# mhx/dwarfs

Measured on AMD Instinct MI355X. Metric: ricepp encode+decode GiB/s, device-resident uint16 blocks, 1/2/4/8 GPUs, higher is better.
Workload: dtype u16; 1 GPU; 4096 independent 64 KiB uint16 blocks per GPU, ricepp bs128 cs1 BE ulsb0, encode+decode round trip (BASELINE.json configs[1]); blocks_per_gpu=4096, block_bytes=65536, parallelism=shard1 (blocks sharded, RCCL all-gather of encoded sizes), step_launch=eager

## Files before the change

### dwarfs_amd/csrc/ricepp_decode_fused.hip

```cpp
#include <hip/hip_runtime.h>
#include <stdint.h>

#include <algorithm>

#include "ricepp_amd.h"
#include "ricepp_internal.h"
#include "ricepp_stats.h"
#include "ricepp_tables.h"

#ifdef RPP_STATS
__device__ unsigned long long g_dec_stats[16];
#endif

namespace {

constexpr int kParsePrio = 1;

__device__ __forceinline__ uint4 tb_entry(const uint4* tb, uint32_t off16) {
  return *reinterpret_cast<const uint4*>(reinterpret_cast<const char*>(tb) + off16);
}

template <uint32_t CS, bool SH>
__global__ __launch_bounds__(kWave* kDecMaxWaves) void rpp_decode_kernel(DecParams p) {
  extern __shared__ __attribute__((aligned(16))) uint4 dsm[];
  const uint32_t b = blockIdx.x * p.waves + __builtin_amdgcn_readfirstlane(threadIdx.x / kWave);
  bool mine = b < p.nblocks;
  if (mine && p.only_fallback) mine = p.status[b] == rpp_internal::kSegFallback;
  if (mine && p.units && p.units[b] > 1) mine = false;
  if (!__syncthreads_or(mine)) return;
  copy_tables(dsm);
  __syncthreads();
  const uint4* tab = dsm;
  const uint32_t lane = lane_id();
  const uint32_t wv = __builtin_amdgcn_readfirstlane(threadIdx.x / kWave);
  uint32_t ring_w = kTabBytes / 4 + wv * kWaveLdsWords;
  asm("" : "+s"(ring_w));
  uint32_t* ring = reinterpret_cast<uint32_t*>(dsm) + ring_w;
  uint32_t* list = ring + kRingWords + kRingPad + kListLead;
  if (lane < kListLead) list[(int)lane - (int)kListLead] = 0u;
  const uint32_t bs = p.bs, be = p.be, ulsb = p.ulsb;
  const uint32_t selbe = be ? 0x02030001u : 0x03020100u;
  const uint32_t selpack = be ? 0x04050001u : 0x05040100u;
  const uint32_t lane24 = kSegBits * lane;
  if (!mine) return;
#ifdef RPP_STATS
  uint32_t stat_acc[16] = {0};
  unsigned long long tprev_;
  asm volatile("s_memtime %0\n\ts_waitcnt lgkmcnt(0)" : "=s"(tprev_)::"memory");
#endif

  int32_t status = RPP_OK;
  uint32_t N = 0, nbytes = 0, mis = 0;
  uint64_t nb_all = 0, lim_all = 0;
  const uint8_t* in = p.in;
  uint16_t* out = p.out;
  {
    const uint64_t n64 = p.n_samples[b];
    const uint64_t ioff = p.in_off[b];
    const uint64_t nb64 = p.in_bytes[b];
    if (n64 % CS != 0 || n64 >= RPP_MAX_STREAM_SAMPLES || nb64 >= (UINT64_C(1) << 32) - 8) {
      status = RPP_INVALID_ARGUMENT;
    } else {
      mis = (uint32_t)(ioff & 3u);
      N = (uint32_t)n64;
      nb_all = nb64 + mis;
      lim_all = 8u * mis + 64u * ((nb64 + 7u) >> 3);
      in = p.in + (ioff - mis);
      out = p.out + p.out_off[b];
    }
  }
  const bool aligned16 = ((uintptr_t)in & 15u) == 0;
  nbytes = (uint32_t)nb_all;
  uint32_t lim = (uint32_t)min(lim_all, (uint64_t)0xFFFFFFFFu);
  uint64_t base_w = 0;
  const uint32_t chunk_len = CS * bs;
  const uint32_t nchunks = status == RPP_OK ? (N + chunk_len - 1) / chunk_len : 0u;

  uint32_t fill_w = 0;
  bool pend = false;
  uint32_t vm_after = 0;
  auto retire = [&]() {
    if (pend) {
      vm_wait_all_but(vm_after);
      fill_w += kChunkWords;
      pend = false;
    }
  };
  auto refill_sync = [&]() {
    const uint32_t w = fill_w + 4 * lane;
    uint4 v;
    if (aligned16 && 4 * w + 16 <= nbytes) {
      v = *reinterpret_cast<const uint4*>(in + 4 * w);
    } else {
      v = make_uint4(stream_word(in, nbytes, w), stream_word(in, nbytes, w + 1), stream_word(in, nbytes, w + 2),
                     stream_word(in, nbytes, w + 3));
    }
    *reinterpret_cast<uint4*>(&ring[w & kRingMask]) = v;
    if ((w & kRingMask) < kRingPad) *reinterpret_cast<uint4*>(&ring[kRingWords + (w & kRingMask)]) = v;
    fill_w += kChunkWords;
  };
  auto request = [&]() {
    if (4u * (fill_w + kChunkWords) > nbytes) return;
    const uint32_t slot = __builtin_amdgcn_readfirstlane((uint32_t)(uintptr_t)&ring[fill_w & kRingMask]);
    const uint8_t* src = in + 4u * fill_w;
    if (aligned16) {
      glds16(src + 16u * lane, slot);
    } else {
#pragma unroll
      for (uint32_t q = 0; q < 4; ++q) glds4(src + 256u * q + 4u * lane, slot + 256u * q);
    }
    if ((fill_w & kRingMask) == 0)
      glds4(src + 4u * lane, __builtin_amdgcn_readfirstlane((uint32_t)(uintptr_t)&ring[kRingWords]));
    pend = true;
    vm_after = 0;
  };
  refill_sync();
  refill_sync();
  lds_fence();
  auto ensure = [&](uint32_t w) {
    if (fill_w < w + kAhead) {
      retire();
      while (fill_w < w + kAhead) refill_sync();
      lds_fence();
    }
  };
  auto wptr = [&](uint32_t w) -> const uint32_t* { return ring + (w & kRingMask); };
  auto peek32 = [&](uint32_t pos) -> uint32_t {
    const uint32_t* q = wptr(pos >> 5);
    return __builtin_amdgcn_alignbit(q[1], q[0], pos & 31u);
  };

  uint32_t last0 = 0, last1 = 0;
  uint32_t P = 8 * mis + 16 * CS;
  auto rebase = [&]() {
    if (P < (1u << 30)) return;
    const uint32_t sh = ((P >> 5) - kRingWords) & ~(kRingWords - 1u);
    in += 4ull * sh;
    base_w += sh;
    P -= 32u * sh;
    fill_w -= sh;
    nbytes = (uint32_t)(nb_all - 4ull * base_w);
    lim = (uint32_t)min(lim_all - 32ull * base_w, (uint64_t)0xFFFFFFFFu);
  };
  if (status == RPP_OK) {
    if (P > lim) status = RPP_TRUNCATED_INPUT;
    last0 = __builtin_amdgcn_readfirstlane(peek32(8 * mis) & 0xFFFFu);
    if (CS > 1) last1 = __builtin_amdgcn_readfirstlane(peek32(8 * mis + 16) & 0xFFFFu);
  }
  auto load_x = [&](uint32_t sb, uint32_t& xl, uint32_t& xh) {
    const uint32_t* q = wptr(sb >> 5);
    const uint32_t o = sb & 31u;
    const uint32_t a0 = q[0], a1 = q[1], a2 = q[2];
    xl = __builtin_amdgcn_alignbit(a1, a0, o);
    xh = __builtin_amdgcn_alignbit(a2, a1, o);
  };
  auto ring_keep = [&](uint32_t q) {
    if (pend && fill_w < (q >> 5) + kAhead + 128) retire();
    if (!pend && fill_w <= (q >> 5) + 766) request();
  };
  const uint32_t nsb = nchunks * CS;
  const bool fast_bs = bs == 2 * kWave ? (CS == 2 || (((uintptr_t)out) & 3u) == 0)
                                       : (bs == 16 || bs == 32 || bs == 64);
  const uint32_t nsb_fast = fast_bs ? (N / chunk_len) * CS : 0u;
  const uint32_t lane_off1 = lane < bs ? 2u * CS * lane : 0x7FFFFFF0u;
  const __amdgpu_buffer_rsrc_t orsrc = __builtin_amdgcn_make_buffer_rsrc(out, (short)0, (int)(2 * N), 0x00020000);
  ScanRegs sreg;

  for (uint32_t s = 0; s < nsb && status == RPP_OK; ++s) {
    rebase();
    auto fast = [&]<uint32_t MT, uint32_t LO, uint32_t HI, bool TWO>() {
      constexpr bool W32 = LO >= 8;
      constexpr uint32_t SB = W32 ? 32u : kSegBits;
      const uint32_t n = TWO ? 2 * kWave : bs;
      const uint4* const list4 = reinterpret_cast<const uint4*>(list);
      uint2* const list2 = reinterpret_cast<uint2*>(list);
      auto seg_bits = [&](uint32_t q, uint32_t& xh) {
        if constexpr (W32) {
          const uint32_t* w = ring + (((q >> 5) + lane) & kRingMask);
          const uint32_t w0 = w[0], w1 = w[1], w2 = w[2];
          xh = __builtin_amdgcn_alignbit(w2, w1, q & 31u);
          return __builtin_amdgcn_alignbit(w1, w0, q & 31u);
        } else {
          const uint32_t x = q + lane24;
          const uint32_t* w = ring + ((x >> 5) & kRingMask);
          xh = 0u;
          return __builtin_amdgcn_alignbit(w[1], w[0], x);
        }
      };
      auto fs_of = [](uint32_t h) { return (h & 15u) - 1u; };
      auto header_ok = [](uint32_t h) { return (uint32_t)((h & 15u) - (LO + 1) <= HI - LO); };
      auto parse = [&](uint32_t q, uint32_t xl, uint32_t xh, uint32_t fs, uint4 e0, uint4 e1, uint4 e2, uint4 e3,
                       uint32_t& Pe, uint32_t& xln, uint32_t& xhn, uint32_t rider, uint32_t& rider_incl,
                       auto&& mid) -> uint32_t {
        __builtin_amdgcn_s_setprio(kParsePrio);
        const uint32_t k = fs + 1;
        const uint32_t pe_base = q + 4u + n * k;
        uint32_t tm, cnt, incl;
        uint32_t tot2;
        if constexpr (!W32) {
          const Map8 M01 = comp8(Map8{e1.x, e1.y}, Map8{e0.x, e0.y});
          const Map8 M = comp8(Map8{e2.x, e2.y}, M01);
          auto scan_sel = [&]() {
            Map8 S = scan8_shr1(M, sreg.r1);
            S = scan8_shr2(S, sreg.r2);
            S = scan8_shr4(S, sreg.r4);
            S = scan8_shr8(S, sreg.r8);
            S = scan8_bc15(S, sreg.b15);
            S = scan8_bc31(S, sreg.b31);
            const Map8 X = shift8_wave(S, sreg.w1);
            return __builtin_amdgcn_perm(X.hi, X.lo, 0xFFFFFF04u);
          };
          auto term_mask = [&](uint32_t sel) {
            const uint32_t a0 = __builtin_amdgcn_perm(e0.w, e0.z, sel);
            const uint32_t a1 = __builtin_amdgcn_perm(e1.w, e1.z, __builtin_amdgcn_perm(e0.y, e0.x, sel));
            const uint32_t a2 = __builtin_amdgcn_perm(e2.w, e2.z, __builtin_amdgcn_perm(M01.hi, M01.lo, sel));
            return __builtin_amdgcn_perm(a2, __builtin_amdgcn_perm(a1, a0, 0x0C0C0400u), 0x0C040100u);
          };
          tm = term_mask(scan_sel());
          cnt = __builtin_popcount(tm);
          const uint32_t incl2 = wave_incl_sum(cnt | (rider << 16));
          incl = incl2 & 0xFFFFu;
          rider_incl = incl2 >> 16;
          tot2 = readlane(incl2, kWave - 1);
        } else {
          uint64_t finm;
          w32_count(e0, e1, e2, e3, n, rider, sreg, tm, cnt, incl, finm, rider_incl);
          tot2 = readlane(incl, kWave - 1) | (readlane(rider_incl, kWave - 1) << 16);
        }
        const uint32_t excl = incl - cnt;
        RPP_TSTAMP(7);
        uint32_t t[MT];
#pragma unroll
        for (uint32_t j = 0; j < MT; ++j) {
          t[j] = ffbl(tm);
          tm &= tm - 1;
        }
        RPP_TSTAMP(8);
        const uint32_t base = cnt != 0 && excl < n ? excl : 256u;
        uint32_t abase = (uint32_t)((int)(SB * lane - 4u) + __mul24((int)base, -(int)k));
        asm volatile("" : "+v"(abase));
        const uint32_t xr = xl >> 1;
#pragma unroll
        for (int j = MT - 1; j >= 0; --j) {
          const uint32_t rem = W32 ? __builtin_amdgcn_ubfe(__builtin_amdgcn_alignbit(xh, xl, t[j]), 1, fs)
                                   : __builtin_amdgcn_ubfe(xr, t[j], fs);
          list2[base + j] = make_uint2(abase + t[j] - j * k, rem);
          lds_fence();
        }
        Pe = pe_base + __builtin_amdgcn_readfirstlane(list[2 * (n - 1)]);
        __builtin_amdgcn_s_setprio(0);
        xln = seg_bits(Pe, xhn);
        mid(rider_incl, tot2 >> 16);
        RPP_TSTAMP(13);
        return (uint32_t)((tot2 & 0xFFFFu) >= n);
      };
      auto deltas = [&](uint4 tt, uint32_t aprev, uint32_t fs, uint32_t& d1, uint32_t& dsum) {
        if constexpr (TWO) {
          const uint32_t df0 = lshl_or(tt.x - aprev, fs, tt.y), df1 = lshl_or(tt.z - tt.x, fs, tt.w);
          const uint32_t d0 = (df0 >> 1) ^ neg_lsb(df0);
          d1 = (df1 >> 1) ^ neg_lsb(df1);
          dsum = d0 + d1;
        } else {
          const uint32_t df = lshl_or(tt.x - aprev, fs, tt.y);
          d1 = (df >> 1) ^ neg_lsb(df);
          dsum = lane < n ? d1 : 0u;
        }
      };
      auto store = [&](uint32_t d1, uint32_t inc, uint32_t inc_last, uint32_t sx) {
        const uint32_t comp = sx % CS;
        const uint32_t lastc = comp ? last1 : last0;
        const uint32_t v1 = lastc + inc;
        if constexpr (!TWO) {
          const uint32_t o = SH ? px_write2<true>(v1, selbe, ulsb) : __builtin_amdgcn_perm(v1, v1, selbe);
          __builtin_amdgcn_raw_buffer_store_b16((uint16_t)o, orsrc, lane_off1,
                                                (int)(2 * ((sx / CS) * chunk_len + comp)), 0);
          const uint32_t lnew = lastc + inc_last;
          if (comp) last1 = lnew;
          else last0 = lnew;
          return;
        }
        const uint32_t o = SH ? px_write2<true>(__builtin_amdgcn_perm(v1, v1 - d1, 0x05040100u), selbe, ulsb)
                              : __builtin_amdgcn_perm(v1, v1 - d1, selpack);
        if constexpr (CS == 1) {
          __builtin_amdgcn_raw_buffer_store_b32(o, orsrc, 4 * lane, (int)(sx * (2 * n)), 0);
        } else {
          const int sbase = (int)(2 * ((sx / CS) * chunk_len + comp));
          __builtin_amdgcn_raw_buffer_store_b16((uint16_t)o, orsrc, 4 * CS * lane, sbase, 0);
          __builtin_amdgcn_raw_buffer_store_b16((uint16_t)(o >> 16), orsrc, 4 * CS * lane + 2 * CS, sbase, 0);
        }
        const uint32_t lnew = lastc + inc_last;
        if (comp) last1 = lnew;
        else last0 = lnew;
      };
      auto lookups = [&](uint32_t xl, uint32_t fs, uint4& e0, uint4& e1, uint4& e2, uint4& e3) {
        const uint4* tb = tab + 256u * fs;
        e0 = tb_entry(tb, sdwa_byte16<0>(xl));
        e1 = tb_entry(tb, sdwa_byte16<1>(xl));
        e2 = tb_entry(tb, sdwa_byte16<2>(xl));
        if constexpr (W32) e3 = tb_entry(tb, sdwa_byte16<3>(xl));
        if constexpr (!W32) e3 = make_uint4(0u, 0u, 0u, 0u);
      };

      uint32_t pn_limit, trig_bits;
      auto ring_bounds = [&]() {
        pn_limit = __builtin_amdgcn_readfirstlane(min(min(lim - 4u, 32u * (fill_w - kAhead) + 31u), 1u << 31));
        trig_bits =
            __builtin_amdgcn_readfirstlane(32u * (pend ? fill_w - (kAhead + 127u) : (fill_w > 766u ? fill_w - 766u : 0u)));
      };
      constexpr uint32_t kStoresPerSub = TWO && CS == 2 ? 2u : 1u;
      uint32_t s_keep = s;
      ring_bounds();
      uint32_t Pn;
      uint32_t xh;
      uint32_t xl = seg_bits(P, xh);
      const uint32_t h = __builtin_amdgcn_readfirstlane(xl);
      uint32_t fs = fs_of(h);
      uint4 e0, e1, e2, e3;
      lookups(xl, fs, e0, e1, e2, e3);
      uint32_t unused_rider;
      uint32_t xlB, xhB;
      uint32_t ok =
          parse(P, xl, xh, fs, e0, e1, e2, e3, Pn, xlB, xhB, 0u, unused_rider, [](uint32_t, uint32_t) {}) & header_ok(h);
      uint32_t pn_read_limit = pn_limit;
      while (ok) {
        uint4 tt;
        uint32_t aprev;
        if constexpr (TWO) {
          tt = list4[lane];
          aprev = list[4 * lane - 2];
        } else {
          const uint2 t2 = list2[lane];
          tt = make_uint4(t2.x, t2.y, 0u, 0u);
          aprev = list[2 * lane - 2];
        }
        const uint32_t hB = __builtin_amdgcn_readfirstlane(xlB);
        RPP_TSTAMP(1);
        RPP_STAT(0, 1);
        uint32_t d1A, sumA, incA;
        const uint32_t nxt = (uint32_t)(s + 1 < nsb_fast) & (uint32_t)(Pn <= pn_read_limit) & header_ok(hB);
        pn_read_limit = pn_limit;
        const uint32_t fsB = fs_of(hB);
        lookups(xlB, fsB, e0, e1, e2, e3);
        deltas(tt, aprev, fs, d1A, sumA);
        RPP_TSTAMP(2);
        uint32_t PnB, xlC, xhC;
        ok = parse(Pn, xlB, xhB, fsB, e0, e1, e2, e3, PnB, xlC, xhC, sumA, incA,
                   [&](uint32_t inc, uint32_t inc_last) { store(d1A, inc, inc_last, s); });
        ++s;
        P = Pn;
        if (!(ok & nxt)) {
          if (P > lim) status = RPP_TRUNCATED_INPUT;
          break;
        }
        Pn = PnB;
        fs = fsB;
        xlB = xlC;
        xhB = xhC;
        if (Pn >= trig_bits) {
          vm_after += (s - s_keep) * kStoresPerSub;
          s_keep = s;
          ring_keep(Pn);
          ring_bounds();
        }
        RPP_TSTAMP(15);
      }
    };
    while (s < nsb_fast && status == RPP_OK && fill_w >= (P >> 5) + kAhead && P + 4 <= lim) {
      rebase();
      const uint32_t* w = ring + ((P >> 5) & kRingMask);
      const uint32_t h = __builtin_amdgcn_readfirstlane(__builtin_amdgcn_alignbit(w[1], w[0], P & 31u)) & 15u;
      const uint32_t s0 = s;
      if (bs == 2 * kWave) {
        if (h - 6u <= 2u) fast.template operator()<4, 5, 7, true>();
        else if (h - 3u <= 2u) fast.template operator()<8, 2, 4, true>();
        else if (h - 9u <= 5u) fast.template operator()<4, 8, 13, true>();
        else if (h == 2u) fast.template operator()<12, 1, 4, true>();
      } else {
        if (h - 6u <= 2u) fast.template operator()<4, 5, 7, false>();
        else if (h - 3u <= 2u) fast.template operator()<8, 2, 4, false>();
        else if (h - 9u <= 5u) fast.template operator()<4, 8, 13, false>();
        else if (h == 2u) fast.template operator()<12, 1, 4, false>();
      }
      last0 &= 0xFFFFu;
      last1 &= 0xFFFFu;
      if (s == s0) break;
    }
    if (s >= nsb || status != RPP_OK) break;
    vm_after = 0;
    const uint32_t comp = s % CS;
    const uint32_t cbase = (s / CS) * chunk_len;
    const uint32_t n = min(N - cbase, chunk_len) / CS;
    RPP_TSTAMP(4);
    ensure(P >> 5);
    if (P + 4 > lim) {
      status = RPP_TRUNCATED_INPUT;
      break;
    }
    uint32_t xl, xh;
    load_x(P + kSegBits * lane, xl, xh);
    const uint32_t fsp1 = __builtin_amdgcn_readfirstlane(xl) & 15u;
    const uint32_t P4 = P + 4;
    uint16_t* dst = out + cbase + comp;
    const bool dw = CS == 1 && (((uintptr_t)dst) & 3u) == 0;
    auto put2 = [&](uint32_t i0, uint32_t o, bool ok0, bool ok1) {
      if (dw && ok1) {
        *reinterpret_cast<uint32_t*>(dst + i0) = o;
      } else {
        if (ok0) dst[CS * i0] = (uint16_t)o;
        if (ok1) dst[CS * (i0 + 1)] = (uint16_t)(o >> 16);
      }
    };
    RPP_STAT(6, 1);
    RPP_TSTAMP(5);
    if (fsp1 == 0) {
      const uint32_t v = px_write(comp ? last1 : last0, be, ulsb) * 0x10001u;
      for (uint32_t i0 = 2 * lane; i0 < n; i0 += 2 * kWave) put2(i0, v, true, i0 + 1 < n);
      P = P4;
    } else if (fsp1 == 15) {
      if ((uint64_t)P4 + 16ull * n > lim) {
        status = RPP_TRUNCATED_INPUT;
        break;
      }
      for (uint32_t i0 = 2 * lane; i0 < n; i0 += 2 * kWave) {
        put2(i0, peek32(P4 + 16 * i0), true, i0 + 1 < n);
      }
      const uint32_t lv = __builtin_amdgcn_readfirstlane(px_read(peek32(P4 + 16 * (n - 1)) & 0xFFFFu, be, ulsb));
      if (comp) last1 = lv;
      else last0 = lv;
      P = P4 + 16 * n;
    } else {
      const uint32_t fs = fsp1 - 1;
      const uint32_t k = fsp1;
      const uint32_t fmask = (1u << fs) - 1u;
      const uint4* tb = tab + 256u * fs;
      uint32_t acc = comp ? last1 : last0, start = P4, xdone = 0;
      uint32_t held_i = 0xFFFFFFFFu, held_r = 0;
      auto extract = [&](uint32_t m) {
        for (; xdone < m; xdone += 2 * kWave) {
          const uint32_t i0 = xdone + 2 * lane;
          const bool ok0 = i0 < m, ok1 = i0 + 1 < m;
          const uint2 tt = *reinterpret_cast<const uint2*>(&list[min(i0, kListDump - 2)]);
          const uint32_t t0 = tt.x, t1 = ok1 ? tt.y : t0;
          const uint32_t st0 = dpp_keep<kDppWaveShr1>(start, t1 + k);
          const uint32_t r0 = i0 == held_i ? held_r : peek32(t0 + 1) & fmask, r1 = peek32(t1 + 1) & fmask;
          const uint32_t df0 = ((t0 - st0) << fs) | r0, df1 = ((t1 - t0 - k) << fs) | r1;
          const uint32_t d0 = ok0 ? (df0 >> 1) ^ (0u - (df0 & 1u)) : 0u;
          const uint32_t d1 = ok1 ? (df1 >> 1) ^ (0u - (df1 & 1u)) : 0u;
          const uint32_t inc = wave_incl_sum(d0 + d1);
          const uint32_t v1 = acc + inc;
          put2(i0, px_write2<true>(((v1 - d1) & 0xFFFFu) | (v1 << 16), selbe, ulsb), ok0, ok1);
          acc += wave_last(inc);
          start = wave_last(t1) + k;
        }
        xdone = m;
        start = __builtin_amdgcn_readfirstlane(list[m - 1]) + k;
      };
      uint32_t q0 = P, s0 = 4, done = 0;
      for (;;) {
        RPP_STAT(0, 1);
        const uint32_t sb = q0 + kSegBits * lane;
        const uint4 e0 = tb[xl & 0xFFu], e1 = tb[__builtin_amdgcn_ubfe(xl, 8, 8)],
                    e2 = tb[__builtin_amdgcn_ubfe(xl, 16, 8)];
        RPP_TSTAMP(10);
        uint32_t tm, xexit;
        if (fs < 8) {
          Map8 M = comp8(Map8{e2.x, e2.y}, comp8(Map8{e1.x, e1.y}, Map8{e0.x, e0.y}));
          M = scan_step8<kDppRowShr1>(M);
          M = scan_step8<kDppRowShr2>(M);
          M = scan_step8<kDppRowShr4>(M);
          M = scan_step8<kDppRowShr8>(M);
          M = scan_step8<kDppRowBcast15, 0xA>(M);
          M = scan_step8<kDppRowBcast31, 0xC>(M);
          const Map8 X{dpp_keep<kDppWaveShr1>(kId0, M.lo), dpp_keep<kDppWaveShr1>(kId1, M.hi)};
          uint32_t sel = __builtin_amdgcn_perm(X.hi, X.lo, s0 | kSelByte0) | kSelByte0;
          const uint32_t t0 = __builtin_amdgcn_perm(e0.w, e0.z, sel);
          sel = __builtin_amdgcn_perm(e0.y, e0.x, sel) | kSelByte0;
          const uint32_t t1 = __builtin_amdgcn_perm(e1.w, e1.z, sel);
          sel = __builtin_amdgcn_perm(e1.y, e1.x, sel) | kSelByte0;
          const uint32_t t2 = __builtin_amdgcn_perm(e2.w, e2.z, sel);
          xexit = __builtin_amdgcn_perm(e2.y, e2.x, sel);
          tm = t0 | (t1 << 8) | (t2 << 16);
        } else {
          const Map16 b0{{e0.x, e0.y, kId0, kId1}}, b1{{e1.x, e1.y, kId0, kId1}}, b2{{e2.x, e2.y, kId0, kId1}};
          Map16 M = comp16(b2, comp16(b1, b0));
          M = scan_step16<kDppRowShr1>(M);
          M = scan_step16<kDppRowShr2>(M);
          M = scan_step16<kDppRowShr4>(M);
          M = scan_step16<kDppRowShr8>(M);
          M = scan_step16<kDppRowBcast15, 0xA>(M);
          M = scan_step16<kDppRowBcast31, 0xC>(M);
          const Map16 X{{dpp_keep<kDppWaveShr1>(kId0, M.w[0]), dpp_keep<kDppWaveShr1>(kId1, M.w[1]),
                         dpp_keep<kDppWaveShr1>(kId2, M.w[2]), dpp_keep<kDppWaveShr1>(kId3, M.w[3])}};
          uint32_t st = sel16(X, s0) & 0xFFu;
          uint32_t t[3];
          const uint4 ee[3] = {e0, e1, e2};
#pragma unroll
          for (int j = 0; j < 3; ++j) {
            const uint32_t sel = st | kSelByte0;
            const bool skip = st >= 8;
            t[j] = skip ? 0u : __builtin_amdgcn_perm(ee[j].w, ee[j].z, sel);
            st = skip ? st - 8 : __builtin_amdgcn_perm(ee[j].y, ee[j].x, sel);
          }
          tm = t[0] | (t[1] << 8) | (t[2] << 16);
          xexit = st;
        }
        RPP_TSTAMP(11);
        const uint32_t cnt = __builtin_popcount(tm);
        const uint32_t incl = wave_incl_sum(cnt);
        const uint32_t excl = incl - cnt;
        const uint32_t need = n - done;
        const uint32_t mine = need > excl ? min(cnt, need - excl) : 0u;
        uint32_t* lp = list + done + excl;
        for (uint32_t j = 0; __any(j < mine); ++j) {
          const uint32_t t = ffbl(tm);
          tm &= tm - 1;
          *(j < mine ? lp + j : list + kListDump) = sb + t;
        }
        RPP_TSTAMP(12);
        if (__ballot(incl >= need)) break;
        done += wave_last(incl);
        if ((done & ~1u) > xdone) {
          lds_fence();
          extract(done & ~1u);
        }
        if ((done & 1u) && held_i != done - 1) {
          lds_fence();
          held_i = done - 1;
          held_r = __builtin_amdgcn_readfirstlane(peek32(list[held_i] + 1)) & fmask;
        }
        s0 = wave_last(xexit);
        q0 += kWinBits;
        if (q0 >= lim) {
          status = RPP_TRUNCATED_INPUT;
          break;
        }
        ensure(q0 >> 5);
        load_x(q0 + kSegBits * lane, xl, xh);
      }
      if (status != RPP_OK) break;
      lds_fence();
      extract(n);
      if (comp) last1 = acc & 0xFFFFu;
      else last0 = acc & 0xFFFFu;
      P = __builtin_amdgcn_readfirstlane(list[n - 1]) + k;
      if (P > lim) {
        status = RPP_TRUNCATED_INPUT;
        break;
      }
    }
    RPP_TSTAMP(14);
    ring_keep(P);
  }
  retire();
  if (lane == 0) p.status[b] = status;
#ifdef RPP_STATS
  if (lane == 0)
    for (int i = 0; i < 16; ++i) atomicAdd(&g_dec_stats[i], (unsigned long long)stat_acc[i]);
#endif
}

}

#ifdef RPP_STATS
extern "C" int rpp_dec_stats_fetch(uint64_t* out, int reset) {
  if (hipMemcpyFromSymbol(out, HIP_SYMBOL(g_dec_stats), sizeof(uint64_t) * 16) != hipSuccess) return RPP_HIP_ERROR;
  if (reset) {
    uint64_t z[16] = {0};
    if (hipMemcpyToSymbol(HIP_SYMBOL(g_dec_stats), z, sizeof z) != hipSuccess) return RPP_HIP_ERROR;
  }
  return RPP_OK;
}
#endif

namespace rpp_internal {

int launch_decode_fused(const rpp_config* cfg, const uint8_t* d_in, const uint64_t* d_in_offsets,
                        const uint64_t* d_in_bytes, uint32_t nblocks, uint16_t* d_out, const uint64_t* d_out_offsets,
                        const uint64_t* d_n_samples, int32_t* d_status, hipStream_t stream, bool only_fallback,
                        const uint64_t* d_units, uint32_t waves, bool rows) {
  int st = rpp_check_config(cfg);
  if (st != RPP_OK) return st;
  if (nblocks == 0) return RPP_OK;
  if (!d_in || !d_in_offsets || !d_in_bytes || !d_out || !d_out_offsets || !d_n_samples || !d_status)
    return RPP_INVALID_ARGUMENT;
  uint32_t W = std::min<uint32_t>(kDecMaxWaves, std::max<uint32_t>(1, (nblocks + 255) / 256));
  if (waves) W = std::min<uint32_t>(kDecMaxWaves, waves);
  const size_t lds = kTabBytes + (size_t)W * kWaveLdsWords * 4;
  static void (*const kernels[4])(DecParams) = {rpp_decode_kernel<1, false>, rpp_decode_kernel<1, true>,
                                                 rpp_decode_kernel<2, false>, rpp_decode_kernel<2, true>};
  static const hipError_t attr_err =
      set_max_dynamic_lds(kernels, kTabBytes + (size_t)kDecMaxWaves * kWaveLdsWords * 4);
  if (attr_err != hipSuccess) return RPP_HIP_ERROR;
  DecParams p{d_in, d_in_offsets, d_in_bytes, d_out, d_out_offsets, d_n_samples, d_status, nblocks,
              cfg->block_size, cfg->component_stream_count, cfg->big_endian ? 1u : 0u,
              cfg->unused_lsb_count, W, only_fallback ? 1u : 0u, d_units};
  const auto k = kernels[2 * (cfg->component_stream_count - 1) + (cfg->unused_lsb_count ? 1 : 0)];
  if (rows && !only_fallback && !d_units && !waves &&
      (cfg->block_size == 16 || cfg->block_size == 32)) {
    st = launch_decode_rows(cfg, d_in, d_in_offsets, d_in_bytes, nblocks, d_out, d_out_offsets, d_n_samples, d_status,
                            stream);
    if (st != RPP_OK) return st;
    p.only_fallback = 1;
  }
  hipLaunchKernelGGL(k, dim3((nblocks + W - 1) / W), dim3(kWave * W), lds, stream, p);
  return hipGetLastError() == hipSuccess ? RPP_OK : RPP_HIP_ERROR;
}

}
```

Baseline: 782.1 GiB/s.

## Add 16-bit segment decode fast path for fs 5..7 with adaptive switching

Measured after the change: 834.0 GiB/s, median of 6. 6.6% higher.

```diff
diff --git a/dwarfs_amd/csrc/ricepp_decode_fused.hip b/dwarfs_amd/csrc/ricepp_decode_fused.hip
--- a/dwarfs_amd/csrc/ricepp_decode_fused.hip
+++ b/dwarfs_amd/csrc/ricepp_decode_fused.hip
@@ -8,6 +8,10 @@
 #include "ricepp_stats.h"
 #include "ricepp_tables.h"
 
+#ifndef RPP_W16
+#define RPP_W16 1
+#endif
+
 #ifdef RPP_STATS
 __device__ unsigned long long g_dec_stats[16];
 #endif
@@ -15,6 +19,10 @@
 namespace {
 
 constexpr int kParsePrio = 1;
+
+constexpr uint32_t kSeg16Bits = 16;
+constexpr uint32_t kWin16Bits = kWave * kSeg16Bits;
+constexpr uint32_t kW16Return = 8;
 
 __device__ __forceinline__ uint4 tb_entry(const uint4* tb, uint32_t off16) {
   return *reinterpret_cast<const uint4*>(reinterpret_cast<const char*>(tb) + off16);
@@ -42,6 +50,7 @@
   const uint32_t selbe = be ? 0x02030001u : 0x03020100u;
   const uint32_t selpack = be ? 0x04050001u : 0x05040100u;
   const uint32_t lane24 = kSegBits * lane;
+  const uint32_t lane16 = kSeg16Bits * lane;
   if (!mine) return;
 #ifdef RPP_STATS
   uint32_t stat_acc[16] = {0};
@@ -165,12 +174,15 @@
   const uint32_t lane_off1 = lane < bs ? 2u * CS * lane : 0x7FFFFFF0u;
   const __amdgpu_buffer_rsrc_t orsrc = __builtin_amdgcn_make_buffer_rsrc(out, (short)0, (int)(2 * N), 0x00020000);
   ScanRegs sreg;
+  uint32_t fit_run = kW16Return;
 
   for (uint32_t s = 0; s < nsb && status == RPP_OK; ++s) {
     rebase();
-    auto fast = [&]<uint32_t MT, uint32_t LO, uint32_t HI, bool TWO>() {
+    auto fast = [&]<uint32_t MT, uint32_t LO, uint32_t HI, bool TWO, bool W16 = false>() {
       constexpr bool W32 = LO >= 8;
-      constexpr uint32_t SB = W32 ? 32u : kSegBits;
+      static_assert(!W16 || (LO >= 5 && HI <= 7 && MT == 3 && TWO), "16-bit segments: fs 5..7, bs 128");
+      constexpr uint32_t SB = W32 ? 32u : W16 ? kSeg16Bits : kSegBits;
+      constexpr bool kCountFit = RPP_W16 != 0 && !W16 && LO == 5 && HI == 7 && TWO;
       const uint32_t n = TWO ? 2 * kWave : bs;
       const uint4* const list4 = reinterpret_cast<const uint4*>(list);
       uint2* const list2 = reinterpret_cast<uint2*>(list);
@@ -181,7 +193,7 @@
           xh = __builtin_amdgcn_alignbit(w2, w1, q & 31u);
           return __builtin_amdgcn_alignbit(w1, w0, q & 31u);
         } else {
-          const uint32_t x = q + lane24;
+          const uint32_t x = q + (W16 ? lane16 : lane24);
           const uint32_t* w = ring + ((x >> 5) & kRingMask);
           xh = 0u;
           return __builtin_amdgcn_alignbit(w[1], w[0], x);
@@ -199,7 +211,7 @@
         uint32_t tot2;
         if constexpr (!W32) {
           const Map8 M01 = comp8(Map8{e1.x, e1.y}, Map8{e0.x, e0.y});
-          const Map8 M = comp8(Map8{e2.x, e2.y}, M01);
+          const Map8 M = W16 ? M01 : comp8(Map8{e2.x, e2.y}, M01);
           auto scan_sel = [&]() {
             Map8 S = scan8_shr1(M, sreg.r1);
             S = scan8_shr2(S, sreg.r2);
@@ -213,6 +225,7 @@
           auto term_mask = [&](uint32_t sel) {
             const uint32_t a0 = __builtin_amdgcn_perm(e0.w, e0.z, sel);
             const uint32_t a1 = __builtin_amdgcn_perm(e1.w, e1.z, __builtin_amdgcn_perm(e0.y, e0.x, sel));
+            if constexpr (W16) return __builtin_amdgcn_perm(a1, a0, 0x0C0C0400u);
             const uint32_t a2 = __builtin_amdgcn_perm(e2.w, e2.z, __builtin_amdgcn_perm(M01.hi, M01.lo, sel));
             return __builtin_amdgcn_perm(a2, __builtin_amdgcn_perm(a1, a0, 0x0C0C0400u), 0x0C040100u);
           };
@@ -296,7 +309,8 @@
         const uint4* tb = tab + 256u * fs;
         e0 = tb_entry(tb, sdwa_byte16<0>(xl));
         e1 = tb_entry(tb, sdwa_byte16<1>(xl));
-        e2 = tb_entry(tb, sdwa_byte16<2>(xl));
+        if constexpr (!W16) e2 = tb_entry(tb, sdwa_byte16<2>(xl));
+        if constexpr (W16) e2 = make_uint4(0u, 0u, 0u, 0u);
         if constexpr (W32) e3 = tb_entry(tb, sdwa_byte16<3>(xl));
         if constexpr (!W32) e3 = make_uint4(0u, 0u, 0u, 0u);
       };
@@ -321,6 +335,9 @@
       uint32_t xlB, xhB;
       uint32_t ok =
           parse(P, xl, xh, fs, e0, e1, e2, e3, Pn, xlB, xhB, 0u, unused_rider, [](uint32_t, uint32_t) {}) & header_ok(h);
+      if constexpr (W16) {
+        if (!ok) fit_run = 0;
+      }
       uint32_t pn_read_limit = pn_limit;
       while (ok) {
         uint4 tt;
@@ -336,8 +353,13 @@
         const uint32_t hB = __builtin_amdgcn_readfirstlane(xlB);
         RPP_TSTAMP(1);
         RPP_STAT(0, 1);
+        if constexpr (W16) RPP_STAT(3, 1);
         uint32_t d1A, sumA, incA;
-        const uint32_t nxt = (uint32_t)(s + 1 < nsb_fast) & (uint32_t)(Pn <= pn_read_limit) & header_ok(hB);
+        uint32_t nxt = (uint32_t)(s + 1 < nsb_fast) & (uint32_t)(Pn <= pn_read_limit) & header_ok(hB);
+        if constexpr (kCountFit) {
+          fit_run = Pn - P <= kWin16Bits ? fit_run + 1 : 0u;
+          nxt &= (uint32_t)(fit_run < kW16Return);
+        }
         pn_read_limit = pn_limit;
         const uint32_t fsB = fs_of(hB);
         lookups(xlB, fsB, e0, e1, e2, e3);
@@ -348,6 +370,9 @@
                    [&](uint32_t inc, uint32_t inc_last) { store(d1A, inc, inc_last, s); });
         ++s;
         P = Pn;
+        if constexpr (W16) {
+          if (!ok) fit_run = 0;
+        }
         if (!(ok & nxt)) {
           if (P > lim) status = RPP_TRUNCATED_INPUT;
           break;
@@ -371,6 +396,12 @@
       const uint32_t h = __builtin_amdgcn_readfirstlane(__builtin_amdgcn_alignbit(w[1], w[0], P & 31u)) & 15u;
       const uint32_t s0 = s;
       if (bs == 2 * kWave) {
+#if RPP_W16
+        if (h - 6u <= 2u && fit_run >= kW16Return) {
+          fast.template operator()<3, 5, 7, true, true>();
+          if (s == s0 && fit_run < kW16Return) continue;
+        } else
+#endif
         if (h - 6u <= 2u) fast.template operator()<4, 5, 7, true>();
         else if (h - 3u <= 2u) fast.template operator()<8, 2, 4, true>();
         else if (h - 9u <= 5u) fast.template operator()<4, 8, 13, true>();
```
